# jedisct1/zig-lz4

Measured on AMD Instinct MI355X. Metric: GiB/s uncompressed, block compress+decompress, higher is better.
Workload: dtype u8

## Files before the change

zig-lz4_amd/csrc/zlz4_compress_fast.hip:

```cpp
#include <cstdlib>

#include "zlz4_device.hpp"

#ifdef ZLZ4_STAMPS
__device__ unsigned long long g_zlz4_stamps[24];
#define STAMP_DECL unsigned long long st_acc[24] = {0,0,0,0,0,0,0,0,0,0,0,0,0,0,0,0,0,0,0,0,0,0,0,0}; unsigned long long st_last = __builtin_amdgcn_s_memtime();
#define STAMP(i) do { unsigned long long st_now; __builtin_amdgcn_sched_barrier(0); \
                      asm volatile("s_memtime %0\n\ts_waitcnt lgkmcnt(0)" : "=s"(st_now) :: "memory"); \
                      __builtin_amdgcn_sched_barrier(0); st_acc[i] += st_now - st_last; st_last = st_now; } while (0)
#define STAMP_COUNT(i) do { st_acc[i] += 1; } while (0)
#define STAMP_FLUSH do { if (lane == 0) for (int st_k = 0; st_k < 24; st_k++) atomicAdd(&g_zlz4_stamps[st_k], st_acc[st_k]); } while (0)
#else
#define STAMP_DECL
#define STAMP(i)
#define STAMP_COUNT(i)
#define STAMP_FLUSH
#endif

namespace zlz4 {

__device__ __forceinline__ uint32_t hash4(uint32_t seq) { return (seq * kHashMul) >> 20; }

__device__ __forceinline__ uint32_t skip_sum(uint32_t x) {
    const uint32_t q = x >> 6, r = x & 63u;
    return 32u * q * (q - 1u) + q * r;
}

__device__ __forceinline__ int64_t emit_last_literals(uint8_t *dst, uint32_t dst_len, uint32_t op,
                                                       const uint8_t *lit_src, uint32_t lit, uint32_t lane) {
    if (lit == 0) return (int64_t)op;
    const uint32_t nle = ext_len_bytes(lit);
    if ((uint64_t)op + 1u + nle + lit > dst_len) return kErrOutputTooSmall;
    if (lane == 0) dst[op] = (uint8_t)((lit >= 15u ? 15u : lit) << 4);
    if (lit >= 15u) write_ext_len(dst + op + 1u, lit, lane);
    copy_bytes(dst + op + 1u + nle, lit_src, lit, lane);
    return (int64_t)(op + 1u + nle + lit);
}

__device__ __forceinline__ uint32_t extend_match(const uint8_t *__restrict__ src, uint32_t m_pos, uint32_t m_cand,
                                                 uint32_t mlen, uint32_t match_limit, uint32_t src_size,
                                                 uint32_t lane) {
    const uint32_t ip0 = m_pos + kMinMatch, mt0 = m_cand + kMinMatch;
    for (;;) {
        const uint32_t p = ip0 + mlen + lane * 16u;
        uint32_t n = 0;
        if (p < match_limit) n = (match_limit - p) < 16u ? (match_limit - p) : 16u;
        uint32_t d = 0;
        if (n > 0) {
            const uint32_t q = mt0 + mlen + lane * 16u;
            if (p + 16u <= src_size) {
                d = first_diff16(ld128(src + p), ld128(src + q));
                if (d > n) d = n;
            } else {
                while (d < n && src[p + d] == src[q + d]) d++;
            }
        }
        const uint64_t stop = ballot(d < 16u);
        if (stop) {
            const uint32_t sl = first_lane(stop);
            return mlen + sl * 16u + rdlane(d, sl);
        }
        mlen += 1024u;
    }
}

template <typename T, int kTag, bool kSeed = false>
__global__ __launch_bounds__(256) void k_compress_fast(
    const uint8_t *__restrict__ d_in, const uint64_t *__restrict__ d_in_off,
    const uint32_t *__restrict__ d_in_len, uint8_t *__restrict__ d_out,
    const uint64_t *__restrict__ d_out_off, const uint32_t *__restrict__ d_out_cap,
    int64_t *__restrict__ d_result, uint32_t nblocks, uint32_t acceleration, uint32_t max_in_len,
    const uint32_t *d_table_in, const uint32_t *__restrict__ d_table_idx, uint32_t *d_table_out) {
    extern __shared__ __attribute__((aligned(16))) uint8_t lds_raw[];
    const uint32_t lane = threadIdx.x & 63u;
    const uint32_t wave_in_wg = threadIdx.x >> 6;
    const uint32_t blk = rfl(blockIdx.x * (blockDim.x >> 6) + wave_in_wg);
    if (blk >= nblocks) return;
    typedef __attribute__((address_space(3))) volatile T lds_entry;
    typedef __attribute__((address_space(3))) volatile uint8_t lds_tag;
    lds_entry *table = (lds_entry *)lds_raw + wave_in_wg * 4096u;
    lds_tag *tags = (lds_tag *)lds_raw + (blockDim.x >> 6) * 4096u * (uint32_t)sizeof(T) + wave_in_wg * 4096u;
    constexpr uint32_t kPosMask = kTag == 2 ? 0x00FFFFFFu : 0xFFFFFFFFu;

    const uint8_t *src = d_in + d_in_off[blk];
    uint8_t *dst = d_out + d_out_off[blk];
    const uint32_t src_size = rfl(d_in_len[blk]);
    const uint32_t dst_len = rfl(d_out_cap[blk]);

    int64_t res;
    if (src_size > kMaxInput) {
        res = kErrInputTooLarge;
    } else if (src_size > max_in_len) {
        res = kErrInvalidState;
    } else if (src_size == 0) {
        res = 0;
    } else if (src_size < kMfLimit + 1u) {
        res = emit_last_literals(dst, dst_len, 0, src, src_size, lane);
    } else {
        if constexpr (kSeed) {
            const uint32_t L = src_size - kMfLimit;
            const uint32_t tix = d_table_idx ? rfl(d_table_idx[blk]) : blk;
            const u32x4 *seed4 = reinterpret_cast<const u32x4 *>(d_table_in + (uint64_t)tix * 4096u);
            for (uint32_t k = lane; k < 1024u; k += 64u) {
                const u32x4 v = seed4[k];
                uint32_t e[4] = {v.x < L ? v.x : 0u, v.y < L ? v.y : 0u, v.z < L ? v.z : 0u, v.w < L ? v.w : 0u};
                if (kTag == 2) {
                    for (int q = 0; q < 4; q++)
                        if (e[q]) e[q] |= ((ld32(src + e[q]) * kHashMul) >> 12 & 0xFFu) << 24;
                }
                for (int q = 0; q < 4; q++) table[4u * k + q] = (T)e[q];
            }
            __builtin_amdgcn_fence(__ATOMIC_RELEASE, "wavefront");
        } else {
        {
            u32x4 z = {0, 0, 0, 0};
            u32x4 *t4 = reinterpret_cast<u32x4 *>(lds_raw) + wave_in_wg * (4096u * sizeof(T) / 16u);
            const uint32_t n16 = 4096u * sizeof(T) / 16u;
            for (uint32_t k = lane; k < n16; k += 64u) t4[k] = z;
        }
        }
        const uint32_t accel = acceleration < 1u ? 1u : (acceleration > 65537u ? 65537u : acceleration);
        const uint32_t cbase = accel > 64u ? accel : 64u;
        const uint32_t s_cbase = skip_sum(cbase);
        const uint32_t L = src_size - kMfLimit;
        const uint32_t match_limit = src_size - kLastLiterals;
        const uint64_t lane_bit = 1ull << lane;
        const uint64_t lanes_below = lane_bit - 1ull;

        uint32_t anchor = 0, op = 0;
        uint32_t F0 = 1;
        bool has_ins = false;
        bool failed = false;
        STAMP_DECL
        STAMP(0);

        uint32_t guard = 0;

        constexpr bool kRing = sizeof(T) == 2;
        uint32_t rpos = 0x80000000u + 4u * lane;
        uint32_t r0 = 0, r1 = 0, r2 = 0;
        uint32_t ring_lim = 0;
        if constexpr (kRing) asm volatile("v_mov_b32 %0, %1" : "=v"(ring_lim) : "s"(src_size - 4u));
        auto ring_q = [&](uint32_t q) -> uint32_t { return q < ring_lim ? q : ring_lim; };
        auto ring_win = [&](uint32_t A) -> uint32_t {
            uint32_t rel = rfl(A - rpos);
            if (rel >= 256u) {
                const bool reload = rel >= 512u;
                const uint32_t nb = reload ? (A & ~127u) + 4u * lane : rpos + 256u;
                asm volatile("s_waitcnt vmcnt(0)\n\t"
                             "s_cmpk_lt_u32 %[rel], 0x200\n\t"
                             "s_cbranch_scc1 1f\n\t"
                             "global_load_dword %[r0], %[q0], %[src]\n\t"
                             "global_load_dword %[r1], %[q1], %[src]\n\t"
                             "s_waitcnt vmcnt(0)\n\t"
                             "s_branch 2f\n"
                             "1:\n\t"
                             "v_mov_b32 %[r0], %[r1]\n\t"
                             "v_mov_b32 %[r1], %[r2]\n"
                             "2:\n\t"
                             "global_load_dword %[r2], %[q2], %[src]"
                             : [r0] "+v"(r0), [r1] "+v"(r1), [r2] "+v"(r2)
                             : [rel] "s"(rel), [q0] "v"(ring_q(nb)), [q1] "v"(ring_q(nb + 256u)), [q2] "v"(ring_q(nb + 512u)),
                               [src] "s"(src)
                             : "scc", "memory");
                rpos = nb;
                rel = reload ? A & 127u : rel - 256u;
            }
            const uint32_t s0 = rel >> 2;
            return shfl(lane >= s0 ? r0 : r1, (s0 + lane) & 63u);
        };
        auto win_bytes = [&](uint32_t W, uint32_t A, uint32_t k0, uint32_t *out, uint32_t n) {
            const uint32_t o = (A & 3u) + lane, jw = (o >> 2) + k0;
            uint32_t lo = shfl(W, jw);
            for (uint32_t k = 0; k < n; k++) {
                const uint32_t hi = shfl(W, jw + k + 1u);
                out[k] = __builtin_amdgcn_alignbyte(hi, lo, o & 3u);
                lo = hi;
            }
        };
        auto ring_fwd = [&](uint32_t W, uint32_t A) -> u32x4 {
            uint32_t d[4];
            win_bytes(W, A, 0u, d, 4u);
            return u32x4{d[0], d[1], d[2], d[3]};
        };
        u32x4 fwd_pf = {0, 0, 0, 0};
        uint32_t w_pf = 0;
        uint32_t pf_anchor = 0xFFFFFFFFu;
        while (F0 < L) {
            if (++guard > src_size) { failed = true; break; }
            int32_t ub = -1;

            if (accel == 1u && F0 == anchor + 1u && (has_ins || anchor == 0u) && (uint64_t)anchor + 192u < L) {
              bool moved = false;
              bool to_generic = false;
              for (;;) {
                const uint32_t A = anchor;
                const uint32_t pos = A + lane;
                const bool wr = has_ins || lane > 0;
                if (kRing && pf_anchor != A) {
                    w_pf = ring_win(A);
                    fwd_pf = ring_fwd(w_pf, A);
                }
                const uint32_t W = w_pf;
                const u32x4 fwd = (kRing || pf_anchor == A) ? fwd_pf : ld128(src + pos);
                const uint32_t prod = fwd.x * kHashMul;
                const uint32_t h = prod >> 20;
                const uint32_t tg = (prod >> 12) & 0xFFu;
                const uint32_t mine = kTag == 2 ? (pos | (tg << 24)) : (uint32_t)(T)pos;
                STAMP(1);
                STAMP_COUNT(16);
                uint32_t old_e = 0, rb = 0, told = tg;
                if (wr) {
                    old_e = table[h];
                    if (kTag == 1) told = tags[h];
                }
                if (kTag == 2) told = old_e >> 24;
                const uint32_t old = old_e & kPosMask;
                const bool old_ok = wr && old > 0 && (!kSeed || old < pos) && (old + kMaxDist >= pos) && (kTag == 0 || told == tg);
                u32x4 cold = {0, 0, 0, 0};
                if (old_ok) cold = ld128(src + old);
                constexpr bool kGuess2 = sizeof(T) == 4;
                const uint32_t old12 = kGuess2 ? shfl(old, (lane + 12u) & 63u) : 0u;
                const bool pred2 = kGuess2 && old_ok && lane < 52u && old12 == old + 12u;
                u32x4 f2 = {0, 0, 0, 0}, c2 = f2, f3 = f2, c3 = f2;
                if (pred2) {
                    if (!kRing) { f2 = ld128(src + pos + 16u); f3 = ld128(src + pos + 32u); }
                    c2 = ld128(src + old + 16u); c3 = ld128(src + old + 32u);
                }
                STAMP(3);
                if (wr) table[h] = (T)mine;
                __builtin_amdgcn_fence(__ATOMIC_RELEASE, "wavefront");
                if (wr) rb = table[h];
                uint64_t losers = ballot(wr && rb != mine);
                uint64_t grp = lane_bit;
                while (losers) {
                    const uint32_t l = first_lane(losers);
                    const uint32_t hh = rdlane(h, l);
                    const uint64_t same = ballot(wr && h == hh);
                    if (wr && h == hh) grp = same;
                    losers &= ~same;
                }
                STAMP(2);

                const bool vo = old_ok && cold.x == fwd.x;
                uint32_t mlo;
                {
                    const uint32_t x1 = fwd.y ^ cold.y, x2 = fwd.z ^ cold.z, x3 = fwd.w ^ cold.w;
                    const uint32_t xs = x1 ? x1 : (x2 ? x2 : x3);
                    const uint32_t xbase = x1 ? 0u : (x2 ? 4u : 8u);
                    mlo = xs ? xbase + ((uint32_t)__builtin_ctz(xs) >> 3) : 12u;
                }
                const bool need2 = vo && mlo == 12u;
                if (need2 && !pred2) {
                    if (!kRing) { f2 = ld128(src + pos + 16u); f3 = ld128(src + pos + 32u); }
                    c2 = ld128(src + old + 16u); c3 = ld128(src + old + 32u);
                }
                if (kRing && ballot(need2)) {
                    uint32_t d[8];
                    win_bytes(W, A, 4u, d, 8u);
                    f2 = u32x4{d[0], d[1], d[2], d[3]};
                    f3 = u32x4{d[4], d[5], d[6], d[7]};
                }
                if (need2) {
                    const uint32_t d2 = first_diff16_sel(f2, c2);
                    mlo += d2 == 16u ? 16u + first_diff16_sel(f3, c3) : d2;
                }
                const bool single = (grp & lanes_below) == 0;
                const bool oldfast = vo && mlo < 44u;
                const uint64_t wrmask = ballot(wr);
                const uint64_t cfast = ballot(oldfast);
                const uint64_t slow = ballot(wr && ((!single && !oldfast) || (vo && mlo >= 44u)));
                const uint64_t nsing = ballot(wr && !single);
                uint32_t J, S;
                {
                    const uint64_t mj = cfast >> lane, ms = slow >> lane;
                    J = mj ? lane + (uint32_t)__builtin_ctzll(mj) : 64u;
                    S = ms ? lane + (uint32_t)__builtin_ctzll(ms) : 64u;
                }
                uint32_t v_end = lane + kMinMatch + mlo;
                uint32_t mlo_e = mlo, off_e = pos - old;
                uint32_t XP, Q;
                {
                    const uint32_t xm = J < S ? J : S;
                    XP = xm | ((uint32_t)((nsing >> (xm & 63u)) & 1ull) << 7);
                    Q = (vo ? 1u : 0u) | (mlo << 1);
                }
                uint32_t PK;
                {
                    const uint32_t jc = J & 63u;
                    const uint32_t ve_j = shfl(v_end, jc);
                    const bool fastok = J < 64u && S > J && !((nsing >> jc) & 1ull);
                    PK = fastok ? (J | (ve_j << 6)) : 0xFFFFFFFFu;
                }

                STAMP(6);
                uint32_t f = 1;
                uint32_t a = 0;
                uint32_t nseq = 0;
                uint64_t covered_x = 0;
                uint64_t mm_win = 0;
                bool continue_generic = false;
                const bool tight = dst_len - op < 512u;
                uint32_t a0 = a, op0 = op;
                uint64_t mm_run = 0;
                auto covered_now = [&]() -> uint64_t {
                    const uint64_t mb = (mm_win | mm_run) & lanes_below;
                    const uint32_t pj = mb ? 63u - (uint32_t)__builtin_clzll(mb) : 0u;
                    const uint32_t pe = shfl(v_end, pj);
                    return covered_x | ballot(mb != 0 && lane < pe);
                };
                auto flush_run = [&]() {
                    STAMP(9); STAMP_COUNT(21);
                    const uint64_t mb = mm_run & lanes_below;
                    const bool has_prev = mb != 0;
                    const uint32_t pj = has_prev ? 63u - (uint32_t)__builtin_clzll(mb) : 0u;
                    const uint32_t pend_all = shfl(v_end, pj);
                    const uint32_t pend = has_prev ? pend_all : a0;
                    const bool cov = has_prev && lane < pend_all;
                    const bool is_m = (mm_run & lane_bit) != 0;
                    const uint32_t jlast = 63u - (uint32_t)__builtin_clzll(mm_run);
                    const bool is_lit = lane >= a0 && lane < jlast && !cov && !is_m;
                    const uint64_t litmask = ballot(is_lit);
                    const uint64_t extm = ballot(is_m && mlo_e >= 15u);
                    const uint64_t at_or_above = mm_run & ~lanes_below;
                    const uint32_t my_m = at_or_above ? (uint32_t)__builtin_ctzll(at_or_above) : lane;
                    const uint32_t own_l = (my_m - pend >= 15u) ? 1u : 0u;
                    const uint64_t lextm = ballot(is_m && own_l != 0u);
                    const uint32_t k = (uint32_t)__popcll(mb);
                    const uint32_t lb = (uint32_t)__popcll(litmask & lanes_below);
                    const uint32_t o1 = op0 + 3u * k + lb + 1u + (uint32_t)__popcll(extm & lanes_below) +
                                        (uint32_t)__popcll(lextm & lanes_below) + own_l;
                    if (is_lit) dst[o1] = (uint8_t)fwd.x;
                    if (is_m) {
                        const uint32_t lit_k = lane - pend;
                        uint8_t *tk = dst + (o1 - 1u - lit_k - own_l);
                        tk[0] = (uint8_t)(((lit_k < 15u ? lit_k : 15u) << 4) | (mlo_e < 15u ? mlo_e : 15u));
                        if (own_l) tk[1] = (uint8_t)(lit_k - 15u);
                        const uint16_t off16 = (uint16_t)off_e;
                        __builtin_memcpy(dst + o1, &off16, 2);
                        if (mlo_e >= 15u) dst[o1 + 2u] = (uint8_t)(mlo_e - 15u);
                    }
                    const uint32_t nm = (uint32_t)__popcll(mm_run);
                    op = op0 + 3u * nm + (uint32_t)__popcll(litmask) + (uint32_t)__popcll(extm) + (uint32_t)__popcll(lextm);
                    mm_win |= mm_run;
                    mm_run = 0;
                    STAMP(10);
                };
                for (;;) {
                    if (mm_run == 0) { a0 = a; op0 = op; }
                    if (!tight) {
                        uint32_t t_pk, t_j;
#define ZLZ4_FAST_RUN_TRIP                                   \
                            "s_cmp_gt_u32 %[f], 63\n\t"      \
                            "s_cbranch_scc1 3f\n\t"          \
                            "v_readlane_b32 %[pk], %[PK], %[f]\n\t" \
                            "s_cmp_eq_u32 %[pk], -1\n\t"     \
                            "s_cbranch_scc1 3f\n\t"          \
                            "s_lshr_b32 %[a], %[pk], 6\n\t"  \
                            "s_add_u32 %[f], %[a], 1\n\t"    \
                            "s_and_b32 %[j], %[pk], 63\n\t"  \
                            "s_bitset1_b64 %[mm], %[j]\n\t"  \
                            "s_add_u32 %[nseq], %[nseq], 1\n\t"
                        asm volatile(
                            "s_nop 3\n"
                            "1:\n\t"
                            ZLZ4_FAST_RUN_TRIP
                            ZLZ4_FAST_RUN_TRIP
                            "s_branch 1b\n"
                            "3:\n"
                            : [f] "+s"(f), [a] "+s"(a), [nseq] "+s"(nseq), [mm] "+s"(mm_run), [pk] "=&s"(t_pk), [j] "=&s"(t_j)
                            : [PK] "v"(PK)
                            : "scc");
#undef ZLZ4_FAST_RUN_TRIP
                    }
                    STAMP(8);
                    if (f >= 64u) {
                        if (nseq == 0u) continue_generic = true;
                        break;
                    }

                    const uint32_t xp = rdlane(XP, f);
                    const uint32_t x = xp & 127u;
                    if (x >= 64u) {
                        if (nseq == 0u) continue_generic = true;
                        break;
                    }
                    uint64_t pm = 0;
                    if (xp >> 7) {
                        const uint64_t grp_x = (uint64_t)rdlane((uint32_t)grp, x) | ((uint64_t)rdlane((uint32_t)(grp >> 32), x) << 32);
                        pm = grp_x & wrmask & ~covered_now() & ((1ull << x) - 1ull);
                    }
                    const uint32_t j = x;
                    const uint32_t m_pos = A + j;
                    uint32_t m_cand, mlen;
                    if (pm) {
                        const uint32_t pr = 63u - (uint32_t)__builtin_clzll(pm);
                        if (rdlane(fwd.x, pr) != rdlane(fwd.x, x)) { STAMP_COUNT(19); STAMP(9); f = x + 1u; continue; }
                        STAMP_COUNT(18);
                        m_cand = A + pr;
                        const uint64_t xa = ((uint64_t)(rdlane(fwd.z, j) ^ rdlane(fwd.z, pr)) << 32) | (rdlane(fwd.y, j) ^ rdlane(fwd.y, pr));
                        const uint32_t xb = rdlane(fwd.w, j) ^ rdlane(fwd.w, pr);
                        if (xa) mlen = (uint32_t)__builtin_ctzll(xa) >> 3;
                        else if (xb) mlen = 8u + ((uint32_t)__builtin_ctz(xb) >> 3);
                        else mlen = extend_match(src, m_pos, m_cand, 12u, match_limit, src_size, lane);
                    } else {
                        const uint32_t q = rdlane(Q, x);
                        if (!(q & 1u)) { STAMP_COUNT(19); STAMP(9); f = x + 1u; continue; }
                        STAMP_COUNT(18);
                        mlen = q >> 1;
                        if (mlen < 44u && !tight) {
                            mm_run |= 1ull << j;
                            nseq++;
                            a = j + kMinMatch + mlen;
                            STAMP(9);
                            if (a >= 64u) break;
                            f = a + 1u;
                            continue;
                        }
                        m_cand = rdlane(old, x);
                        if (mlen >= 44u) mlen = extend_match(src, m_pos, m_cand, 44u, match_limit, src_size, lane);
                    }
                    const uint32_t lit = j - a;
                    const uint32_t offset = m_pos - m_cand;
                    const uint32_t e = j + kMinMatch + mlen;
                    if (!tight && mlen < 270u) {
                        v_end = wrlane(e, j, v_end);
                        mlo_e = wrlane(mlen, j, mlo_e);
                        off_e = wrlane(offset, j, off_e);
                        mm_run |= 1ull << j;
                        nseq++;
                        a = e;
                        STAMP(9);
                        if (e >= 64u) break;
                        f = e + 1u;
                        continue;
                    }
                    if (mm_run) flush_run();
                    const uint32_t nle = ext_len_bytes(lit), nme = ext_len_bytes(mlen);
                    const uint64_t seq_end = (uint64_t)op + 1u + nle + lit + 2u + nme;
                    if (seq_end > dst_len) { failed = true; break; }
                    if (lane == 0)
                        dst[op] = (uint8_t)(((lit >= 15u ? 15u : lit) << 4) | (mlen >= 15u ? 15u : mlen));
                    if (lit >= 15u) write_ext_len(dst + op + 1u, lit, lane);
                    uint8_t *o = dst + op + 1u + nle;
                    if (lane >= a && lane < j) o[lane - a] = (uint8_t)fwd.x;
                    o += lit;
                    if (lane < 2u) o[lane] = (uint8_t)(offset >> (8u * lane));
                    if (mlen >= 15u) write_ext_len(o + 2u, mlen, lane);
                    op = (uint32_t)seq_end;
                    {
                        const uint64_t upto_e = e >= 64u ? ~0ull : (1ull << e) - 1ull;
                        covered_x |= upto_e & ~((2ull << j) - 1ull);
                    }
                    nseq++;
                    a = e;
                    if (e >= 64u) break;
                    f = e + 1u;
                }
                const bool next_win = !continue_generic && !failed && a != 0u && (uint64_t)A + a + 192u < L;
                if (next_win) {
                    pf_anchor = A + a;
                    if constexpr (kRing) {
                        w_pf = ring_win(pf_anchor);
                        fwd_pf = ring_fwd(w_pf, pf_anchor);
                    } else {
                        fwd_pf = ld128(src + pf_anchor + lane);
                    }
                }
                if (mm_run && !failed) flush_run();
                anchor = A + a;
                STAMP(4);
                const uint32_t f_end = continue_generic ? 64u : (a >= 64u ? 64u : a + 1u);
                const uint64_t ins = wrmask & ~covered_now() & (f_end >= 64u ? ~0ull : (1ull << f_end) - 1ull);
                if (failed) break;
                if (wr && !(ins & lane_bit)) table[h] = (T)old_e;
                __builtin_amdgcn_fence(__ATOMIC_RELEASE, "wavefront");
                if ((ins & lane_bit) && (grp & ins & ~lanes_below & ~lane_bit) == 0) {
                    table[h] = (T)mine;
                    if (kTag == 1) tags[h] = (uint8_t)tg;
                }
                __builtin_amdgcn_fence(__ATOMIC_RELEASE, "wavefront");
                STAMP(5);
                moved = anchor != A;
                to_generic = continue_generic;
                if (next_win) {
                    has_ins = true;
                    F0 = anchor + 1u;
                    if (++guard > src_size) { failed = true; break; }
                    continue;
                }
                break;
              }
                if (failed) break;
                if (!to_generic && moved) {
                    if (anchor < L) { has_ins = true; F0 = anchor + 1u; }
                    else { has_ins = false; F0 = L; }
                    continue;
                }
                if (to_generic) ub = 63;
            }

            bool found = false, bailed = false;
            uint32_t m_pos = 0, m_cand = 0, m_local = 0;
            bool m_local_done = false;
            for (;;) {
                const int32_t u = ub + (int32_t)lane;
                uint32_t pos, step_next;
                if (u <= 0) {
                    pos = (u < 0) ? F0 - 1u : F0;
                    step_next = accel;
                } else if (u == 1) {
                    pos = F0 + accel;
                    step_next = accel >> 6;
                } else {
                    const uint32_t x = cbase + (uint32_t)u - 1u;
                    pos = F0 + accel + skip_sum(x) - s_cbase;
                    step_next = x >> 6;
                }
                const bool is_probe = u >= 0;
                const bool bail = is_probe && ((uint64_t)pos + step_next > L);
                const uint64_t bail_mask = ballot(bail);
                const uint32_t nb = bail_mask ? first_lane(bail_mask) : 64u;
                const bool active = (lane < nb) && (is_probe || has_ins);

                const bool have16 = active && (pos + 16u <= src_size);
                u32x4 fwd = {0, 0, 0, 0};
                if (have16) fwd = ld128(src + pos);
                else if (active) fwd.x = ld32(src + pos);
                const uint32_t prod = fwd.x * kHashMul;
                const uint32_t h = prod >> 20;
                const uint32_t tg = (prod >> 12) & 0xFFu;
                const uint32_t mine = kTag == 2 ? (pos | (tg << 24)) : (uint32_t)(T)pos;

                uint32_t old_e = 0, rb = 0, told = tg;
                if (active) {
                    old_e = table[h];
                    if (kTag == 1) told = tags[h];
                    table[h] = (T)mine;
                }
                if (kTag == 2) told = old_e >> 24;
                const uint32_t old = old_e & kPosMask;
                __builtin_amdgcn_fence(__ATOMIC_RELEASE, "wavefront");
                if (active) rb = table[h];
                uint64_t losers = ballot(active && rb != mine);
                uint64_t grp = lane_bit;
                int32_t pred = -1;
                while (losers) {
                    const uint32_t l = first_lane(losers);
                    const uint32_t hh = rdlane(h, l);
                    const uint64_t same = ballot(active && h == hh);
                    if (active && h == hh) {
                        grp = same;
                        const uint64_t below = same & lanes_below;
                        pred = below ? 63 - (int32_t)__clzll((long long)below) : -1;
                    }
                    losers &= ~same;
                }
                const uint32_t pred_pos = shfl(pos, (uint32_t)(pred < 0 ? 0 : pred));
                const uint32_t cand = pred >= 0 ? pred_pos : old;

                bool valid = is_probe && active && cand > 0 && cand < pos && (cand + kMaxDist >= pos) &&
                             (kTag == 0 || pred >= 0 || told == tg);
                u32x4 cnd = {0, 0, 0, 0};
                if (valid) {
                    if (have16) cnd = ld128(src + cand); else cnd.x = ld32(src + cand);
                    valid = cnd.x == fwd.x;
                }
                const uint64_t valid_mask = ballot(valid);

                if (valid_mask) {
                    const uint32_t wl = first_lane(valid_mask);
                    if (active && lane > wl) table[h] = (T)old_e;
                    __builtin_amdgcn_fence(__ATOMIC_RELEASE, "wavefront");
                    const uint64_t upto = (2ull << wl) - 1ull;
                    if (active && lane <= wl && ((grp & upto & ~lanes_below & ~lane_bit) == 0)) {
                        table[h] = (T)mine;
                        if (kTag == 1) tags[h] = (uint8_t)tg;
                    }
                    uint32_t loc = 0;
                    bool loc_done = false;
                    if (lane == wl) {
                        const uint32_t lim = match_limit - (pos + kMinMatch);
                        if (have16) {
                            u32x4 a = fwd, b = cnd;
                            a.x = 0; b.x = 0;
                            loc = first_diff16(a, b) - 4u;
                            if (loc >= lim) { loc = lim; loc_done = true; }
                            else if (loc < 12u) loc_done = true;
                        }
                    }
                    m_pos = rdlane(pos, wl);
                    m_cand = rdlane(cand, wl);
                    m_local = rdlane(loc, wl);
                    m_local_done = rdlane((uint32_t)loc_done, wl) != 0;
                    found = true;
                    break;
                }
                if (bail_mask) {
                    if constexpr (kSeed) {
                        if (active && ((grp & ~lanes_below & ~lane_bit) == 0) && grp != lane_bit) table[h] = (T)mine;
                        __builtin_amdgcn_fence(__ATOMIC_RELEASE, "wavefront");
                    }
                    bailed = true; break;
                }
                if (active && ((grp & ~lanes_below & ~lane_bit) == 0)) {
                    if (grp != lane_bit) table[h] = (T)mine;
                    if (kTag == 1) tags[h] = (uint8_t)tg;
                }
                __builtin_amdgcn_fence(__ATOMIC_RELEASE, "wavefront");
                ub += 64;
            }
            if (bailed || !found) break;
            STAMP_COUNT(20);

            const uint32_t mlen = m_local_done ? m_local
                                               : extend_match(src, m_pos, m_cand, m_local, match_limit, src_size, lane);

            const uint32_t lit = m_pos - anchor;
            const uint32_t nle = ext_len_bytes(lit), nme = ext_len_bytes(mlen);
            const uint64_t seq_end = (uint64_t)op + 1u + nle + lit + 2u + nme;
            if (seq_end > dst_len) { failed = true; break; }
            if (lane == 0)
                dst[op] = (uint8_t)(((lit >= 15u ? 15u : lit) << 4) | (mlen >= 15u ? 15u : mlen));
            if (lit >= 15u) write_ext_len(dst + op + 1u, lit, lane);
            uint8_t *o = dst + op + 1u + nle;
            copy_bytes(o, src + anchor, lit, lane);
            o += lit;
            const uint32_t offset = m_pos - m_cand;
            if (lane < 2u) o[lane] = (uint8_t)(offset >> (8u * lane));
            if (mlen >= 15u) write_ext_len(o + 2u, mlen, lane);
            op = (uint32_t)seq_end;

            const uint32_t end = m_pos + kMinMatch + mlen;
            anchor = end;
            if (end < L) { has_ins = true; F0 = end + 1u; }
            else { has_ins = false; F0 = L; }
        }
        if constexpr (kRing) asm volatile("s_waitcnt vmcnt(0)" : "+v"(r2));
        if constexpr (kSeed) {
            if (!failed && has_ins && F0 >= L && lane == 0) {
                const uint32_t prod = ld32(src + anchor) * kHashMul;
                table[prod >> 20] = (T)(kTag == 2 ? (anchor | ((prod >> 12 & 0xFFu) << 24)) : anchor);
            }
        }
        res = failed ? kErrOutputTooSmall
                     : emit_last_literals(dst, dst_len, op, src + anchor, src_size - anchor, lane);
        STAMP(7);
        STAMP_FLUSH;
    }
    if constexpr (kSeed) {
        if (d_table_out) {
            const uint32_t tix = d_table_idx ? rfl(d_table_idx[blk]) : blk;
            const uint32_t *seed = d_table_in + (uint64_t)tix * 4096u;
            uint32_t *out = d_table_out + (uint64_t)blk * 4096u;
            const bool merged = src_size >= kMfLimit + 1u && src_size <= max_in_len && src_size <= kMaxInput && res >= 0;
            if (merged) {
                const uint32_t L = src_size - kMfLimit;
                __builtin_amdgcn_fence(__ATOMIC_RELEASE, "wavefront");
                for (uint32_t k = lane; k < 4096u; k += 64u) {
                    const uint32_t v = seed[k];
                    const uint32_t loaded = v < L ? v : 0u;
                    const uint32_t f = (uint32_t)table[k] & kPosMask;
                    out[k] = f != loaded ? f : v;
                }
            } else if (out != seed) {
                const u32x4 *s4 = reinterpret_cast<const u32x4 *>(seed);
                u32x4 *o4 = reinterpret_cast<u32x4 *>(out);
                for (uint32_t k = lane; k < 1024u; k += 64u) o4[k] = s4[k];
            }
        }
    }
    if (lane == 0) d_result[blk] = res;
}

__global__ __launch_bounds__(256) void k_load_dict(const uint8_t *__restrict__ d_dict, const uint64_t *__restrict__ d_dict_off,
                                                   const uint32_t *__restrict__ d_dict_len, uint32_t *__restrict__ d_tables,
                                                   int64_t *__restrict__ d_result, uint32_t ndicts) {
    __shared__ uint32_t t[4096];
    const uint32_t d = blockIdx.x;
    if (d >= ndicts) return;
    const uint32_t lane = threadIdx.x & 63u;
    const uint32_t len = d_dict_len[d];
    const uint32_t size = len < 65536u ? len : 65536u;
    const uint8_t *tail = d_dict + d_dict_off[d] + (len - size);
    for (uint32_t k = threadIdx.x; k < 4096u; k += blockDim.x) t[k] = 0;
    __syncthreads();
    if (size >= kMinMatch) {
        const uint32_t n = size - kMinMatch;
        for (uint32_t base = threadIdx.x - lane; base < n; base += blockDim.x) {
            const uint32_t i = base + lane;
            const bool act = i < n;
            const uint32_t h = act ? hash4(ld32(tail + i)) : 0xFFFFFFFFu;
            const uint32_t hr = shfl(h, lane + 1u);
            if (act && !(lane < 63u && hr == h)) atomicMax(&t[h], i);
        }
    }
    __syncthreads();
    uint32_t *out = d_tables + (uint64_t)d * 4096u;
    for (uint32_t k = threadIdx.x; k < 4096u; k += blockDim.x) out[k] = t[k];
    if (threadIdx.x == 0) d_result[d] = (int64_t)size;
}

}

extern "C" int zlz4_launch_compress_fast(hipStream_t stream, const uint8_t *d_in, const uint64_t *d_in_off,
                                         const uint32_t *d_in_len, uint8_t *d_out, const uint64_t *d_out_off,
                                         const uint32_t *d_out_cap, int64_t *d_result, uint32_t nblocks,
                                         uint32_t max_in_len, uint32_t acceleration) {
    if (nblocks == 0) return 0;
    static const uint32_t lds_pad = [] { const char *e = zlz4_tune_env("ZLZ4_TUNE_LDS_PAD"); return e ? (uint32_t)atoi(e) : 0u; }();
    static const uint32_t tune_wpw = [] { const char *e = zlz4_tune_env("ZLZ4_TUNE_WPW"); return e ? (uint32_t)atoi(e) : 0u; }();
    static const int tune_tag = [] { const char *e = zlz4_tune_env("ZLZ4_TUNE_TAG"); return e ? atoi(e) : -1; }();
#define ZLZ4_LAUNCH_FAST(KERN, T, TAG, WPW, LDS)                                                                      \
    hipLaunchKernelGGL((zlz4::KERN<T, TAG>), dim3((nblocks + (WPW) - 1) / (WPW)), dim3(64 * (WPW)), (LDS),              \
                       stream, d_in, d_in_off, d_in_len, d_out, d_out_off, d_out_cap, d_result, nblocks, acceleration,  \
                       max_in_len, nullptr, nullptr, nullptr)
    if (max_in_len <= 65536u + 11u) {
        const uint32_t wpw = (tune_wpw == 2 || tune_wpw == 4) ? tune_wpw : 1;
        if (tune_tag > 0) ZLZ4_LAUNCH_FAST(k_compress_fast, uint16_t, 1, wpw, wpw * (4096 * sizeof(uint16_t) + 4096) + lds_pad);
        else ZLZ4_LAUNCH_FAST(k_compress_fast, uint16_t, 0, wpw, wpw * 4096 * sizeof(uint16_t) + lds_pad);
    } else {
        const uint32_t wpw = (tune_wpw == 2) ? 2 : 1;
        if (tune_tag != 0 && max_in_len <= (1u << 24)) ZLZ4_LAUNCH_FAST(k_compress_fast, uint32_t, 2, wpw, wpw * 4096 * sizeof(uint32_t) + lds_pad);
        else ZLZ4_LAUNCH_FAST(k_compress_fast, uint32_t, 0, wpw, wpw * 4096 * sizeof(uint32_t) + lds_pad);
    }
#undef ZLZ4_LAUNCH_FAST
    return hipGetLastError() == hipSuccess ? 0 : -7;
}

extern "C" int zlz4_launch_compress_fast_continue(hipStream_t stream, const uint8_t *d_in, const uint64_t *d_in_off,
                                                  const uint32_t *d_in_len, uint8_t *d_out, const uint64_t *d_out_off,
                                                  const uint32_t *d_out_cap, const uint32_t *d_table_in,
                                                  const uint32_t *d_table_idx, uint32_t *d_table_out, int64_t *d_result,
                                                  uint32_t nblocks, uint32_t max_in_len, uint32_t acceleration) {
    if (nblocks == 0) return 0;
    static const int tune_tag = [] { const char *e = zlz4_tune_env("ZLZ4_TUNE_TAG"); return e ? atoi(e) : -1; }();
#define ZLZ4_LAUNCH_SEEDED(T, TAG)                                                                                      \
    hipLaunchKernelGGL((zlz4::k_compress_fast<T, TAG, true>), dim3(nblocks), dim3(64), 4096 * sizeof(T), stream, d_in,   \
                       d_in_off, d_in_len, d_out, d_out_off, d_out_cap, d_result, nblocks, acceleration, max_in_len,      \
                       d_table_in, d_table_idx, d_table_out)
    if (max_in_len <= 65536u + 11u) ZLZ4_LAUNCH_SEEDED(uint16_t, 0);
    else if (tune_tag != 0 && max_in_len <= (1u << 24)) ZLZ4_LAUNCH_SEEDED(uint32_t, 2);
    else ZLZ4_LAUNCH_SEEDED(uint32_t, 0);
#undef ZLZ4_LAUNCH_SEEDED
    return hipGetLastError() == hipSuccess ? 0 : -7;
}

extern "C" int zlz4_launch_load_dict(hipStream_t stream, const uint8_t *d_dict, const uint64_t *d_dict_off,
                                     const uint32_t *d_dict_len, uint32_t *d_tables, int64_t *d_result, uint32_t ndicts) {
    if (ndicts == 0) return 0;
    hipLaunchKernelGGL(zlz4::k_load_dict, dim3(ndicts), dim3(256), 0, stream, d_dict, d_dict_off, d_dict_len, d_tables,
                       d_result, ndicts);
    return hipGetLastError() == hipSuccess ? 0 : -7;
}

#ifdef ZLZ4_STAMPS
extern "C" int zlz4_debug_read_stamps(unsigned long long *out16, int reset) {
    if (hipMemcpyFromSymbol(out16, HIP_SYMBOL(g_zlz4_stamps), 24 * sizeof(unsigned long long)) != hipSuccess) return -7;
    if (reset) {
        unsigned long long z[24] = {0};
        if (hipMemcpyToSymbol(HIP_SYMBOL(g_zlz4_stamps), z, sizeof z) != hipSuccess) return -7;
    }
    return 0;
}
#endif
```

Before: 81.22.

## Precompute nearest same-hash predecessor match info per lane before serial scan

Before the serial match-selection loop, each lane in a non-singleton hash-collision group now finds its nearest lower group member. It computes whether their first 4 bytes match and how far they extend (up to 12 bytes), and packs this into a per-lane word D1. In the serial loop, when that predecessor is not covered by an earlier match, the packed result is used directly. This replaces the per-step readlanes of grp and fwd fields and the recomputed XOR/ctz chain. It adds wave-wide shuffles to every iteration that has collisions, and it relies on the covered_x/mm_win/v_end logic to decide correctly whether the nearest predecessor is still available.

```diff
diff --git a/zig-lz4_amd/csrc/zlz4_compress_fast.hip b/zig-lz4_amd/csrc/zlz4_compress_fast.hip
--- a/zig-lz4_amd/csrc/zlz4_compress_fast.hip
+++ b/zig-lz4_amd/csrc/zlz4_compress_fast.hip
@@ -241,6 +241,19 @@
                     losers &= ~same;
                 }
                 STAMP(2);
+                const bool single = (grp & lanes_below) == 0;
+                const uint64_t nsing = ballot(wr && !single);
+                uint32_t D1 = 0;
+                if (nsing) {
+                    const uint64_t gb = grp & lanes_below;
+                    const uint32_t p1 = gb ? 63u - (uint32_t)__builtin_clzll(gb) : 0u;
+                    const uint32_t g0 = shfl(fwd.x, p1), g1 = shfl(fwd.y, p1), g2 = shfl(fwd.z, p1), g3 = shfl(fwd.w, p1);
+                    const uint32_t x1 = fwd.y ^ g1, x2 = fwd.z ^ g2, x3 = fwd.w ^ g3;
+                    const uint32_t xs = x1 ? x1 : (x2 ? x2 : x3);
+                    const uint32_t xbase = x1 ? 0u : (x2 ? 4u : 8u);
+                    const uint32_t ext = xs ? xbase + ((uint32_t)__builtin_ctz(xs) >> 3) : 12u;
+                    D1 = p1 | (g0 == fwd.x ? 64u : 0u) | (ext << 7) | ((gb & (gb - 1ull)) == 0 ? 2048u : 0u);
+                }
 
                 const bool vo = old_ok && cold.x == fwd.x;
                 uint32_t mlo;
@@ -265,12 +278,10 @@
                     const uint32_t d2 = first_diff16_sel(f2, c2);
                     mlo += d2 == 16u ? 16u + first_diff16_sel(f3, c3) : d2;
                 }
-                const bool single = (grp & lanes_below) == 0;
                 const bool oldfast = vo && mlo < 44u;
                 const uint64_t wrmask = ballot(wr);
                 const uint64_t cfast = ballot(oldfast);
                 const uint64_t slow = ballot(wr && ((!single && !oldfast) || (vo && mlo >= 44u)));
-                const uint64_t nsing = ballot(wr && !single);
                 uint32_t J, S;
                 {
                     const uint64_t mj = cfast >> lane, ms = slow >> lane;
@@ -386,14 +397,32 @@
                         break;
                     }
                     uint64_t pm = 0;
+                    uint32_t d1 = 0;
                     if (xp >> 7) {
-                        const uint64_t grp_x = (uint64_t)rdlane((uint32_t)grp, x) | ((uint64_t)rdlane((uint32_t)(grp >> 32), x) << 32);
-                        pm = grp_x & wrmask & ~covered_now() & ((1ull << x) - 1ull);
+                        const uint32_t dx = rdlane(D1, x);
+                        const uint32_t p1 = dx & 63u;
+                        const uint64_t mb1 = (mm_win | mm_run) & ((1ull << p1) - 1ull);
+                        bool p1_put = !((covered_x >> p1) & 1ull);
+                        if (p1_put && mb1) p1_put = p1 >= rdlane(v_end, 63u - (uint32_t)__builtin_clzll(mb1));
+                        if (p1_put) {
+                            d1 = dx | 4096u;
+                        } else if (!(dx & 2048u)) {
+                            STAMP_COUNT(14);
+                            const uint64_t grp_x = (uint64_t)rdlane((uint32_t)grp, x) | ((uint64_t)rdlane((uint32_t)(grp >> 32), x) << 32);
+                            pm = grp_x & wrmask & ~covered_now() & ((1ull << x) - 1ull);
+                        }
                     }
                     const uint32_t j = x;
                     const uint32_t m_pos = A + j;
                     uint32_t m_cand, mlen;
-                    if (pm) {
+                    if (d1) {
+                        STAMP_COUNT(12);
+                        if (!(d1 & 64u)) { STAMP_COUNT(19); STAMP(9); f = x + 1u; continue; }
+                        STAMP_COUNT(18);
+                        m_cand = A + (d1 & 63u);
+                        mlen = (d1 >> 7) & 15u;
+                        if (mlen == 12u) mlen = extend_match(src, m_pos, m_cand, 12u, match_limit, src_size, lane);
+                    } else if (pm) {
                         const uint32_t pr = 63u - (uint32_t)__builtin_clzll(pm);
                         if (rdlane(fwd.x, pr) != rdlane(fwd.x, x)) { STAMP_COUNT(19); STAMP(9); f = x + 1u; continue; }
                         STAMP_COUNT(18);
```

New measurement: 80.25. -1.2%, worse.
